# graphdeco-inria/hierarchical-3d-gaussians

Hardware: AMD Instinct MI355X
Metric: fwd+bwd frames/s @1080p, 1M Gaussians (higher is better)
Workload: dtype f32

## Files before the change

hierarchical-3d-gaussians_amd/csrc/preprocess.hip:

```cpp
#include "gaussian_math.h"
#include "half_widen.h"

#include <stdlib.h>

#include <mutex>

namespace hgs {

namespace {

struct CamLds {
  float vm[16];
  float pm[16];
  float cam[3];
};

__device__ __forceinline__ void load_camera(const hgs_raster_args& a, CamLds& c) {
#pragma unroll
  for (int i = 0; i < 16; ++i) {
    c.vm[i] = a.viewmatrix[i];
    c.pm[i] = a.projmatrix[i];
  }
  c.cam[0] = a.campos[0];
  c.cam[1] = a.campos[1];
// ... 826 lines not shown
    for (int i = 0; i < 10; ++i) t[i] = 0.0;
#pragma unroll 4
    for (uint32_t k = (uint32_t)lane; k < r1 - r0; k += 64u) {
      const float2 v0 = ip[k * 5 + 0], v1 = ip[k * 5 + 1], v2 = ip[k * 5 + 2], v3 = ip[k * 5 + 3], v4 = ip[k * 5 + 4];
      t[0] += v0.x; t[1] += v0.y; t[2] += v1.x; t[3] += v1.y;
      t[4] += v2.x; t[5] += v2.y; t[6] += v3.x; t[7] += v3.y;
      t[8] += v4.x; t[9] += v4.y;
    }
#pragma unroll
    for (int i = 0; i < 10; ++i) red[i * 64 + lane] = t[i];
    __builtin_amdgcn_fence(__ATOMIC_RELEASE, "wavefront");
    __builtin_amdgcn_wave_barrier();
    __builtin_amdgcn_fence(__ATOMIC_ACQUIRE, "wavefront");
    if (lane < 40) {
      double acc = 0.0;
      const double* src = red + (lane >> 2) * 64 + (lane & 3) * 16;
#pragma unroll
      for (int j = 0; j < 16; ++j) acc += src[j];
      red[640 + lane] = acc;
    }
    __builtin_amdgcn_fence(__ATOMIC_RELEASE, "wavefront");
    __builtin_amdgcn_wave_barrier();
    __builtin_amdgcn_fence(__ATOMIC_ACQUIRE, "wavefront");
    if (lane < 10) {
      const double* q = red + 640 + lane * 4;
      reinterpret_cast<double*>(inst + rbase * kInstStride)[lane] = ((q[0] + q[1]) + q[2]) + q[3];
    }
    __builtin_amdgcn_fence(__ATOMIC_RELEASE, "wavefront");
    __builtin_amdgcn_wave_barrier();
  }
}

constexpr uint32_t kK8StageRec = 256;
__device__ __forceinline__ void k8_sum_runs(const GeomWs& g, const float* __restrict__ inst, int idx, uint32_t n,
                                            int presummed, float2* st, double (&s)[10]) {
  const int lane = threadIdx.x & 63;
  const unsigned long long long_mask = presummed ? __ballot(n > kK8LongRun) : 0ull;
  if (long_mask == 0ull) {
    uint32_t incl = n;
#pragma unroll
    for (int off = 1; off < 64; off <<= 1) {
      const uint32_t t = __shfl_up(incl, off, 64);
      if (lane >= off) incl += t;
    }
    const uint32_t my0 = incl - n, my1 = incl;
    const uint32_t total = __shfl(incl, 63, 64);
    if (total) {
      const unsigned long long nz = __ballot(n != 0u);
      const int first = __ffsll((long long)nz) - 1;
      const uint32_t off_mine = n ? g.offsets[idx] : 0u;
      const size_t base = (size_t)__shfl(off_mine, first, 64);
      for (uint32_t c0 = 0; c0 < total; c0 += kK8StageRec) {
        const uint32_t cn = min(kK8StageRec, total - c0) * 5u;
        const float2* src = reinterpret_cast<const float2*>(inst) + (base + c0) * 5;
        for (uint32_t t0 = 0; t0 < cn; t0 += 64u * 4u) {
          float2 v[4];
#pragma unroll
          for (int j = 0; j < 4; ++j) {
            const uint32_t t = t0 + (uint32_t)j * 64u + (uint32_t)lane;
            v[j] = src[min(t, cn - 1u)];
          }
#pragma unroll
          for (int j = 0; j < 4; ++j) {
            const uint32_t t = t0 + (uint32_t)j * 64u + (uint32_t)lane;
            if (t < cn) st[t] = v[j];
          }
        }
        __builtin_amdgcn_fence(__ATOMIC_RELEASE, "wavefront");
        __builtin_amdgcn_wave_barrier();
        __builtin_amdgcn_fence(__ATOMIC_ACQUIRE, "wavefront");
        const uint32_t k0 = max(my0, c0), k1 = min(my1, c0 + kK8StageRec);
        for (uint32_t k = k0; k < k1; ++k) {
          const float2* r = st + (k - c0) * 5u;
          const float2 v0 = r[0], v1 = r[1], v2 = r[2], v3 = r[3], v4 = r[4];
          s[0] += v0.x; s[1] += v0.y; s[2] += v1.x; s[3] += v1.y;
          s[4] += v2.x; s[5] += v2.y; s[6] += v3.x; s[7] += v3.y;
          s[8] += v4.x; s[9] += v4.y;
        }
        __builtin_amdgcn_fence(__ATOMIC_RELEASE, "wavefront");
        __builtin_amdgcn_wave_barrier();
      }
    }
  } else if (n != 0u) {
    const size_t off = (size_t)g.offsets[idx];
    if (n > kK8LongRun) {
      const uint32_t nseg = k8_nseg(n);
      for (uint32_t j = 0; j < nseg; ++j) {
        const double* ps = reinterpret_cast<const double*>(inst + (off + (size_t)j * kK8Seg) * kInstStride);
#pragma unroll
        for (int i = 0; i < 10; ++i) s[i] += ps[i];
      }
    } else {
      const float2* ip = reinterpret_cast<const float2*>(inst) + off * 5;
#pragma unroll 2
      for (uint32_t k = 0; k < n; ++k) {
        const float2 v0 = ip[k * 5 + 0], v1 = ip[k * 5 + 1], v2 = ip[k * 5 + 2], v3 = ip[k * 5 + 3], v4 = ip[k * 5 + 4];
        s[0] += v0.x; s[1] += v0.y; s[2] += v1.x; s[3] += v1.y;
        s[4] += v2.x; s[5] += v2.y; s[6] += v3.x; s[7] += v3.y;
        s[8] += v4.x; s[9] += v4.y;
      }
    }
  }
}

template <bool LOD>
__device__ __forceinline__ void k8_chain(const hgs_raster_args& a, const GeomWs& g, int idx, const double (&s)[10],
                                         float (&p)[3], float (&d_mean)[3], float (&d_m2)[3], float& d_op,
                                         float (&d_scale)[3], float (&d_rot)[4], float (&d_c3)[6], float (&gr)[3]) {
  CamLds cam;
  load_camera(a, cam);
  gr[0] = (float)s[6]; gr[1] = (float)s[7]; gr[2] = (float)s[8];
  const uint32_t flags = g.flags[idx];
  load_mean<LOD>(a, lod_row_gather<LOD>(a, idx), p);
  float q[4] = {1.f, 0.f, 0.f, 0.f};
  float sc[3] = {1.f, 1.f, 1.f};
  double qnorm = 1.0;
  ProjD pd;
  if (a.cov3D_precomp) {
#pragma unroll
    for (int i = 0; i < 6; ++i) pd.c3[i] = (double)a.cov3D_precomp[(size_t)idx * 6 + i];
  } else {
    load_scale_rot<LOD>(a, idx, sc, q, &qnorm);
    cov3d_from_scale_rot_d(sc, a.scale_modifier, q, pd);
  }
  project_gaussian_d(p, cam.vm, cam.pm, a.width, a.height, a.tanfovx, a.tanfovy, (flags & 8u) != 0,
                     (flags & 16u) != 0, pd);

  const double A = pd.conA, B = pd.conB, C = pd.conC;
  const double gA = -0.5 * s[2], gB = -s[3], gC = -0.5 * s[4];
  const double ggx = -(A * s[0] + B * s[1]);
  const double ggy = -(C * s[1] + B * s[0]);
  const double dm2x = ggx * 0.5 * (double)a.width, dm2y = ggy * 0.5 * (double)a.height;
  d_m2[0] = (float)dm2x;
  d_m2[1] = (float)dm2y;
  double dmean[3] = {0.0, 0.0, 0.0};

  const double dhx = dm2x * pd.pw, dhy = dm2y * pd.pw;
  const double dhw = -(dm2x * pd.hx + dm2y * pd.hy) * pd.pw * pd.pw;
#pragma unroll
  for (int j = 0; j < 3; ++j)
    dmean[j] += (double)cam.pm[j * 4 + 0] * dhx + (double)cam.pm[j * 4 + 1] * dhy + (double)cam.pm[j * 4 + 3] * dhw;

  const double a2 = pd.a, b2 = pd.b, c2 = pd.c;
  const double di2 = pd.di * pd.di;
  const double ga = (-c2 * c2 * gA + b2 * c2 * gB - b2 * b2 * gC) * di2;
  const double gb = (2.0 * b2 * c2 * gA - (a2 * c2 + b2 * b2) * gB + 2.0 * a2 * b2 * gC) * di2;
  const double gc = (-b2 * b2 * gA + a2 * b2 * gB - a2 * a2 * gC) * di2;
  const double hb = 0.5 * gb;
  double Gs[3][3];
#pragma unroll
  for (int i = 0; i < 3; ++i)
#pragma unroll
    for (int j = i; j < 3; ++j)
      Gs[i][j] = Gs[j][i] = pd.T0[i] * (ga * pd.T0[j] + hb * pd.T1[j]) + pd.T1[i] * (hb * pd.T0[j] + gc * pd.T1[j]);
  d_c3[0] = (float)Gs[0][0];
// ... 47 lines not shown
#pragma unroll
    for (int k = 0; k < 3; ++k) {
      double acc = 0.0;
#pragma unroll
      for (int i = 0; i < 3; ++i) {
        acc += R[i * 3 + k] * dM[i][k];
        gR[i][k] = dM[i][k] * sv[k];
      }
      double dsk = (double)a.scale_modifier * acc;
      if (a.activations & HGS_ACT_SCALE_EXP) dsk *= (double)sc[k];
      d_scale[k] = (float)dsk;
    }
    const double r = q[0], x = q[1], y = q[2], z = q[3];
    double dq[4];
    dq[0] = 2.0 * (-z * gR[0][1] + y * gR[0][2] + z * gR[1][0] - x * gR[1][2] - y * gR[2][0] + x * gR[2][1]);
    dq[1] = 2.0 * (y * gR[0][1] + z * gR[0][2] + y * gR[1][0] - 2.0 * x * gR[1][1] - r * gR[1][2] +
                   z * gR[2][0] + r * gR[2][1] - 2.0 * x * gR[2][2]);
    dq[2] = 2.0 * (-2.0 * y * gR[0][0] + x * gR[0][1] + r * gR[0][2] + x * gR[1][0] + z * gR[1][2] -
                   r * gR[2][0] + z * gR[2][1] - 2.0 * y * gR[2][2]);
    dq[3] = 2.0 * (-2.0 * z * gR[0][0] - r * gR[0][1] + x * gR[0][2] + r * gR[1][0] - 2.0 * z * gR[1][1] +
                   y * gR[1][2] + x * gR[2][0] + y * gR[2][1]);
    if (a.activations & HGS_ACT_ROT_NORMALIZE) {
      const double dot = r * dq[0] + x * dq[1] + y * dq[2] + z * dq[3];
      const double inv = 1.0 / qnorm;
      dq[0] = (dq[0] - r * dot) * inv; dq[1] = (dq[1] - x * dot) * inv;
      dq[2] = (dq[2] - y * dot) * inv; dq[3] = (dq[3] - z * dot) * inv;
    }
    d_rot[0] = (float)dq[0]; d_rot[1] = (float)dq[1]; d_rot[2] = (float)dq[2]; d_rot[3] = (float)dq[3];
  }

  {
    float dod = 1.0f;
    double dact = 1.0;
    const float o_act = load_opacity<LOD>(a, idx, &dact);
    float o_rec = o_act;
    if (a.interpolation_weights && a.num_node_kids && !a.lod_per_pixel)
      o_rec = lod_opacity(o_act, a.interpolation_weights[idx], a.num_node_kids[idx], &dod);
    const float sums5 = o_rec > 0.0f ? (float)(s[5] / (double)o_rec) : 0.0f;
    d_op = a.activations ? (float)((double)sums5 * (double)dod * dact) : sums5 * dod;
  }

  if (!a.colors_precomp) {
    if (flags & 1u) gr[0] = 0.f;
    if (flags & 2u) gr[1] = 0.f;
    if (flags & 4u) gr[2] = 0.f;
  }
}

template <bool ACC>
__device__ __forceinline__ void k8_store_row(const hgs_raster_grads& out, int idx, const float (&d_m2)[3], float d_op,
                                             const float (&d_scale)[3], const float (&d_rot)[4], const float (&d_c3)[6],
                                             const float (&d_col)[3]) {
  constexpr bool acc = ACC;
#pragma unroll
  for (int j = 0; j < 3; ++j) out.dL_dmeans2D[idx * 3 + j] = d_m2[j];
  out.dL_dopacity[idx] = d_op + (acc ? out.dL_dopacity[idx] : 0.f);
  if (out.dL_dcolors) {
#pragma unroll
    for (int j = 0; j < 3; ++j) out.dL_dcolors[idx * 3 + j] = d_col[j];
  }
  if (out.dL_dscales) {
#pragma unroll
    for (int j = 0; j < 3; ++j) out.dL_dscales[idx * 3 + j] = d_scale[j] + (acc ? out.dL_dscales[idx * 3 + j] : 0.f);
  }
  if (out.dL_drotations) {
    float4* dst = reinterpret_cast<float4*>(out.dL_drotations) + idx;
    float4 v = make_float4(d_rot[0], d_rot[1], d_rot[2], d_rot[3]);
    if (acc) { const float4 o = *dst; v.x += o.x; v.y += o.y; v.z += o.z; v.w += o.w; }
    *dst = v;
  }
  if (out.dL_dcov3D) {
#pragma unroll
    for (int j = 0; j < 6; ++j) out.dL_dcov3D[(size_t)idx * 6 + j] = d_c3[j] + (acc ? out.dL_dcov3D[(size_t)idx * 6 + j] : 0.f);
  }
}

template <bool ACC, bool LOD>
__global__ __launch_bounds__(kPreBlock) void preprocess_bwd_kernel(hgs_raster_args a, GeomWs g,
                                                                   const float* __restrict__ inst,
                                                                   float* __restrict__ drgb,
                                                                   float* __restrict__ dmean_rows,
                                                                   const uint32_t* __restrict__ lod_flag,
                                                                   hgs_raster_grads out, int presummed) {
  const int idx = blockIdx.x * kPreBlock + threadIdx.x;
  const bool in_range = idx < a.P;
  const uint32_t n = in_range ? g.tiles_touched[idx] : 0u;

  double s[10];
#pragma unroll
  for (int i = 0; i < 10; ++i) s[i] = 0.0;
  static_assert(kInstStride == 10, "instance record = the ten sums, 40 bytes");
  __shared__ float2 stage[kPreBlock / 64][kK8StageRec * 5];
  k8_sum_runs(g, inst, idx, n, presummed, stage[threadIdx.x >> 6], s);
  if constexpr (!LOD) {
    if (!in_range) return;
  }

  float d_mean[3] = {0.f, 0.f, 0.f};
  float d_m2[3] = {0.f, 0.f, 0.f};
  float d_op = 0.f;
  float d_scale[3] = {0.f, 0.f, 0.f};
  float d_rot[4] = {0.f, 0.f, 0.f, 0.f};
  float d_c3[6] = {0.f, 0.f, 0.f, 0.f, 0.f, 0.f};
  float gr[3] = {0.f, 0.f, 0.f};
  float d_col[3] = {0.f, 0.f, 0.f};
  if (n != 0) {
    float p[3];
    k8_chain<LOD>(a, g, idx, s, p, d_mean, d_m2, d_op, d_scale, d_rot, d_c3, gr);
    if (a.colors_precomp) {
      d_col[0] = gr[0]; d_col[1] = gr[1]; d_col[2] = gr[2];
    } else {
      drgb[idx * 3 + 0] = gr[0];
      drgb[idx * 3 + 1] = gr[1];
      drgb[idx * 3 + 2] = gr[2];
    }
  }

  if constexpr (LOD) {
    if (a.lod_scatter) {
      __shared__ float lds_v[8 * kPreBlock];
      __shared__ int lds_par[kPreBlock];
      __shared__ unsigned char lds_vis[kPreBlock];
      const int t = threadIdx.x;
      const int block_first = blockIdx.x * kPreBlock;
      const int count = min(kPreBlock, a.P - block_first);
      LodRow l;
      l.r = l.p = 0; l.w = 1.0f; l.u = 0.0f;
      if (in_range) l = lod_row<true>(a, idx);
      const bool self = l.p == l.r;
      const bool vis = in_range && n != 0;
      const float wn = self ? 1.0f : l.w, u = (self || !vis) ? 0.0f : l.u;
      float sgn = 1.0f;
      if (vis && !self && u != 0.0f) {
        const float4 qa = reinterpret_cast<const float4*>(a.rotations)[l.r];
        const float4 qb = reinterpret_cast<const float4*>(a.rotations)[l.p];
        sgn = (qa.x * qb.x + qa.y * qb.y + qa.z * qb.z + qa.w * qb.w) < 0.0f ? -1.0f : 1.0f;
      }
      if (in_range) {
#pragma unroll
        for (int j = 0; j < 3; ++j) {
          dmean_rows[idx * 3 + j] = d_mean[j];
          out.dL_dmeans2D[idx * 3 + j] = d_m2[j];
        }
      }
      if (vis) {
        out.dL_dopacity[l.r] = wn * d_op;
#pragma unroll
        for (int j = 0; j < 3; ++j) out.dL_dscales[l.r * 3 + j] = wn * d_scale[j];
        reinterpret_cast<float4*>(out.dL_drotations)[l.r] = make_float4(wn * d_rot[0], wn * d_rot[1], wn * d_rot[2], wn * d_rot[3]);
      }
      lds_par[t] = in_range ? (int)l.p : -1;
      lds_vis[t] = (vis && !self) ? 1 : 0;
#pragma unroll
      for (int j = 0; j < 3; ++j) lds_v[j * kPreBlock + t] = u * d_scale[j];
#pragma unroll
      for (int j = 0; j < 4; ++j) lds_v[(3 + j) * kPreBlock + t] = (u * sgn) * d_rot[j];
      lds_v[7 * kPreBlock + t] = u * d_op;
      __syncthreads();
      if (t < count) {
        const LodRun run = lod_run(a, lds_par, t, count, block_first, *lod_flag != 0u);
        if (run.leader) {
          float acc8[8] = {0.f, 0.f, 0.f, 0.f, 0.f, 0.f, 0.f, 0.f};
          bool any = false;
          for (int j = t; j < run.end; ++j) {
            if (!lds_vis[j]) continue;
            any = true;
#pragma unroll
            for (int k = 0; k < 8; ++k) acc8[k] += lds_v[k * kPreBlock + j];
          }
          if (any) {
            const size_t pp = (size_t)lds_par[t];
#pragma unroll
            for (int k = 0; k < 3; ++k) lod_add(out.dL_dscales + pp * 3 + k, acc8[k], run.atomic);
#pragma unroll
            for (int k = 0; k < 4; ++k) lod_add(out.dL_drotations + pp * 4 + k, acc8[3 + k], run.atomic);
            lod_add(out.dL_dopacity + pp, acc8[7], run.atomic);
          }
        }
      }
      return;
    }
    if (!in_range) return;
  }
#pragma unroll
  for (int j = 0; j < 3; ++j) out.dL_dmeans3D[idx * 3 + j] = d_mean[j] + (ACC ? out.dL_dmeans3D[idx * 3 + j] : 0.f);
  k8_store_row<ACC>(out, idx, d_m2, d_op, d_scale, d_rot, d_c3, d_col);
}


template <bool ACC, bool JAC, bool LOD>
__global__ __launch_bounds__(kPreBlock) void sh_bwd_kernel(hgs_raster_args a, GeomWs g,
                                                           const float* __restrict__ drgb,
                                                           const float* __restrict__ dmean_rows,
                                                           const uint32_t* __restrict__ lod_flag, hgs_raster_grads out) {
  extern __shared__ __attribute__((aligned(16))) unsigned char smem_raw[];
  float* lds = reinterpret_cast<float*>(smem_raw);
  const int n = a.M * 3;
  const bool split = a.shs_rest != nullptr;
  const bool coop = (n & 3) == 0;
  const int block_first = blockIdx.x * kPreBlock;
  const int idx = block_first + threadIdx.x;
  const bool valid = idx < a.P;
  const bool active = valid && g.tiles_touched[idx] != 0;
  if (!JAC && coop) {
    if (split) {
      coop_load_seg(a.shs, block_first, a.P, 3, 0, sh_row_stride(n), lds);
      coop_load_seg(a.shs_rest, block_first, a.P, n - 3, 3, sh_row_stride(n), lds);
    } else {
      coop_load_sh(a.shs, block_first, a.P, n, lds);
    }
    __syncthreads();
  }
  float dsh[48];
#pragma unroll
  for (int i = 0; i < 48; ++i) dsh[i] = 0.f;
  float sh[JAC ? 1 : 48];
  if constexpr (!JAC) {
    if (active) {
      if (coop) lds_row_read(lds, n, sh);
// ... 143 lines not shown
    float* d1 = out.dL_dshs_rest + (size_t)idx * (n - 3);
#pragma unroll
    for (int i = 0; i < 48; ++i) {
      if (i < 3) d0[i] = dsh[i] + (ACC ? d0[i] : 0.f);
      else if (i < n) d1[i - 3] = dsh[i] + (ACC ? d1[i - 3] : 0.f);
    }
  } else if (valid) {
    if (ACC) {
      const float* old = out.dL_dshs + (size_t)idx * n;
#pragma unroll
      for (int i = 0; i < 48; ++i)
        if (i < n) dsh[i] += old[i];
    }
    store_sh(out.dL_dshs, idx, a.M, dsh);
  }
}

__device__ __forceinline__ float k8_dot3(float x0, float y0, float x1, float y1, float x2, float y2) {
#pragma clang fp contract(off)
  return __fmaf_rn(x2, y2, __fmaf_rn(x0, y0, x1 * y1));
}
__device__ __forceinline__ void k8_add_view_term(const float (&gr)[3], const float (&J)[9], float ux, float uy, float uz,
                                                 float inv, float (&d_mean)[3]) {
#pragma clang fp contract(off)
  const float gdx = k8_dot3(gr[0], J[0], gr[1], J[1], gr[2], J[2]);
  const float gdy = k8_dot3(gr[0], J[3], gr[1], J[4], gr[2], J[5]);
  const float gdz = k8_dot3(gr[0], J[6], gr[1], J[7], gr[2], J[8]);
  const float dot = k8_dot3(ux, gdx, uy, gdy, uz, gdz);
  d_mean[0] = __fmaf_rn(__fmaf_rn(-ux, dot, gdx), inv, d_mean[0] + 0.f);
  d_mean[1] = __fmaf_rn(__fmaf_rn(-uy, dot, gdy), inv, d_mean[1] + 0.f);
  d_mean[2] = __fmaf_rn(__fmaf_rn(-uz, dot, gdz), inv, d_mean[2] + 0.f);
}

__global__ __launch_bounds__(kPreBlock) void preprocess_bwd_sh_kernel(hgs_raster_args a, GeomWs g,
                                                                         const float* __restrict__ inst,
                                                                         hgs_raster_grads out, int presummed) {
  extern __shared__ __attribute__((aligned(16))) unsigned char smem_raw[];
  const int block_first = blockIdx.x * kPreBlock;
  const int idx = block_first + threadIdx.x;
  const bool in_range = idx < a.P;
  const uint32_t n = in_range ? g.tiles_touched[idx] : 0u;

  double s[10];
#pragma unroll
  for (int i = 0; i < 10; ++i) s[i] = 0.0;
  k8_sum_runs(g, inst, idx, n, presummed, reinterpret_cast<float2*>(smem_raw) + (threadIdx.x >> 6) * (kK8StageRec * 5), s);

  float d_mean[3] = {0.f, 0.f, 0.f};
  float d_m2[3] = {0.f, 0.f, 0.f};
  float d_op = 0.f;
  float d_scale[3] = {0.f, 0.f, 0.f};
  float d_rot[4] = {0.f, 0.f, 0.f, 0.f};
  float d_c3[6] = {0.f, 0.f, 0.f, 0.f, 0.f, 0.f};
  float gr[3] = {0.f, 0.f, 0.f};
  float b[16];
  const int nb = (a.sh_degree + 1) * (a.sh_degree + 1);
  float p[3];
  if (n != 0) k8_chain<false>(a, g, idx, s, p, d_mean, d_m2, d_op, d_scale, d_rot, d_c3, gr);
  if (in_range) {
    const float d_col[3] = {0.f, 0.f, 0.f};
    k8_store_row<false>(out, idx, d_m2, d_op, d_scale, d_rot, d_c3, d_col);
  }
  __builtin_amdgcn_sched_barrier(0);
  if (n != 0) {
    float ux, uy, uz;
    const float inv = unit_dir(p, a.campos, ux, uy, uz);
    sh_basis(a.sh_degree, ux, uy, uz, b);
    const float* jp = g.shjac + (size_t)idx * kJacStride;
    float J[9];
#pragma unroll
    for (int k = 0; k < 9; ++k) J[k] = jp[k];
    k8_add_view_term(gr, J, ux, uy, uz, inv, d_mean);
  } else {
#pragma unroll
    for (int j = 0; j < 3; ++j) d_mean[j] = 0.f;
  }
  if (in_range) {
#pragma unroll
    for (int j = 0; j < 3; ++j) out.dL_dmeans3D[idx * 3 + j] = d_mean[j];
  }

  float* lds = reinterpret_cast<float*>(smem_raw);
  const int nc = a.M * 3, stride = sh_row_stride(nc);
  __syncthreads();
  if (in_range) {
    float* row = lds + threadIdx.x * stride;
#pragma unroll
    for (int i = 0; i < 12; ++i) {
      if (i * 4 < nc) {
        float v[4];
#pragma unroll
        for (int c = 0; c < 4; ++c) {
          const int k = (i * 4 + c) / 3, ch = (i * 4 + c) % 3;
          v[c] = (n != 0 && k < nb) ? b[k] * gr[ch] : 0.f;
        }
        *reinterpret_cast<float4*>(row + i * 4) = make_float4(v[0], v[1], v[2], v[3]);
      }
    }
  }
  __syncthreads();
  coop_store_sh<false>(out.dL_dshs, block_first, a.P, nc, lds);
}

template <bool ACC, bool COOP, bool COLOR>
__device__ __forceinline__ void sh_bwd_batched_body(const ShBwdViews& v, int P, int M, int sh_degree,
                                                    const float* __restrict__ means3D, const float* __restrict__ shs,
                                                    float* __restrict__ dL_dshs, float* __restrict__ dL_dmeans3D) {
  extern __shared__ __attribute__((aligned(16))) unsigned char smem_raw[];
  float* lds = reinterpret_cast<float*>(smem_raw);
  const int n = M * 3;
  constexpr bool coop = COOP;
  const int block_first = blockIdx.x * kPreBlock;
// ... 250 lines not shown
              : h48   ? (jac ? preprocess_fwd_h48_kernel<true> : preprocess_fwd_h48_kernel<false>)
              : defer ? (jac ? preprocess_fwd_kernel<true, false, true> : preprocess_fwd_kernel<false, false, true>)
                      : (jac ? preprocess_fwd_kernel<true, false, false> : preprocess_fwd_kernel<false, false, false>);
    hipLaunchKernelGGL(k1, dim3(nblk), dim3(kPreBlock), lds_bytes, s, a, g, radii, super, heavy_thr);
    HGS_LAUNCH_CHECK("preprocess_fwd", s, a.debug);
  }
  return HGS_OK;
}

int launch_scan_block_sums(const GeomWs& g, int32_t P, hipStream_t s, bool debug, uint32_t* total_mirror) {
  const int nblk = (P + kPreBlock - 1) / kPreBlock;
  const int chunks = scan_chunks(nblk), resident = scan_resident_workgroups();
  if (chunks * (1 + kBands) <= resident && !scan_split_forced()) {
    hipLaunchKernelGGL(scan_block_sums_kernel, dim3(chunks, 1 + kBands), dim3(1024), 0, s, g.block_sums, g.block_band,
                       nblk, g.scan_chain, total_mirror, 0, chunks);
    HGS_LAUNCH_CHECK("scan_block_sums", s, debug);
    return HGS_OK;
  }
  for (int y = 0; y < 1 + kBands; ++y) {
    uint32_t* sums = y == 0 ? g.block_sums : g.block_band + (size_t)(y - 1) * (nblk + 1);
    for (int c0 = 0; c0 < chunks; c0 += resident) {
      hipLaunchKernelGGL(scan_block_sums_kernel, dim3(min(resident, chunks - c0), 1), dim3(1024), 0, s, sums, g.block_band,
                         nblk, g.scan_chain + (size_t)y * chunks, y == 0 ? total_mirror : nullptr, c0, chunks);
      HGS_LAUNCH_CHECK("scan_block_sums", s, debug);
    }
  }
  return HGS_OK;
}

int launch_preprocess_bwd(const hgs_raster_args& a, const GeomWs& g, const BwdWs& w, const hgs_raster_grads& out, uint32_t L,
                          hipStream_t s) {
  const int nblk = (a.P + kPreBlock - 1) / kPreBlock;
  if (nblk > 0) {
    static const char* force = getenv("HGS_K8_PRESUM");
    const bool presum = force ? force[0] == '1' : (uint64_t)L > 6ull * (uint64_t)a.P;
    if (presum) {
      HGS_HIP(hipMemsetAsync(w.work_counter, 0, sizeof(uint32_t), s));
      hipLaunchKernelGGL(k8_worklist_kernel, dim3(nblk < kWorklistGrid ? nblk : kWorklistGrid), dim3(kPreBlock), 0, s, a.P,
                         g.tiles_touched, w.work, w.work_counter);
      HGS_LAUNCH_CHECK("preprocess_bwd_worklist", s, a.debug);
      const int want = (int)(((size_t)L / 64 + 3) / 4);
      hipLaunchKernelGGL(k8_presum_work_kernel, dim3(want < 1 ? 1 : (want < kPresumGrid ? want : kPresumGrid)), dim3(kPreBlock), 0,
                         s, w.work, w.work_counter, g.tiles_touched, g.offsets, w.inst_grads);
      HGS_LAUNCH_CHECK("preprocess_bwd_long_runs", s, a.debug);
    }
    const char* fuse_env = getenv("HGS_K8_FUSE");
    const bool fused = !(fuse_env && fuse_env[0] == '0') && !a.lod_render_indices && !a.accumulate_grads &&
                       !a.defer_sh_bwd && a.shs && !a.shs_rest && out.dL_dshs && a.prepare_backward && !a.colors_precomp &&
                       ((a.M * 3) & 3) == 0;
    if (fused) {
      const size_t stage_bytes = (size_t)(kPreBlock / 64) * kK8StageRec * 5 * sizeof(float2);
      const size_t rows_bytes = (size_t)kPreBlock * (a.M * 3 + 4) * sizeof(float);
      hipLaunchKernelGGL(preprocess_bwd_sh_kernel, dim3(nblk), dim3(kPreBlock),
                         stage_bytes > rows_bytes ? stage_bytes : rows_bytes, s, a, g, w.inst_grads, out, presum ? 1 : 0);
      HGS_LAUNCH_CHECK("preprocess_bwd_sh", s, a.debug);
      return HGS_OK;
    }
    auto k8a = a.lod_render_indices ? preprocess_bwd_kernel<false, true>
                                    : (a.accumulate_grads ? preprocess_bwd_kernel<true, false> : preprocess_bwd_kernel<false, false>);
    hipLaunchKernelGGL(k8a, dim3(nblk), dim3(kPreBlock), 0, s, a, g, w.inst_grads, w.drgb, w.dmean_rows, w.lod_flag, out,
                       presum ? 1 : 0);
    HGS_LAUNCH_CHECK("preprocess_bwd", s, a.debug);
    if (a.shs && out.dL_dshs && !a.defer_sh_bwd) {
      const size_t lds_bytes = (size_t)kPreBlock * (a.M * 3 + 4) * sizeof(float);
      auto k8b = a.lod_render_indices ? sh_bwd_kernel<false, true, true>
                 : (a.prepare_backward && a.shs) ? (a.accumulate_grads ? sh_bwd_kernel<true, true, false> : sh_bwd_kernel<false, true, false>)
                                                 : (a.accumulate_grads ? sh_bwd_kernel<true, false, false> : sh_bwd_kernel<false, false, false>);
      hipLaunchKernelGGL(k8b, dim3(nblk), dim3(kPreBlock), lds_bytes, s, a, g, w.drgb, w.dmean_rows, w.lod_flag, out);
      HGS_LAUNCH_CHECK("sh_bwd", s, a.debug);
    }
  }
  return HGS_OK;
}

}
```

Measured before the change: 1529.

## Stage backward preprocess inputs and instance grads into LDS via direct global-to-LDS loads

Adds a staged variant of the per-Gaussian backward preprocess kernels. Per-instance gradient records, per-Gaussian means, scales, rotations, opacity, flags and the SH Jacobian rows are loaded into LDS with global_load_lds (buffer-to-LDS DMA) instead of going through VGPRs. The camera load is hoisted to kernel entry and the row store in the fused kernel is moved to the end, so the loads can overlap the summation. The new path raises LDS use per block, which may reduce occupancy. It also depends on 16-byte alignment checks, shifted-offset arithmetic and explicit vmcnt waits.

```diff
diff --git a/hierarchical-3d-gaussians_amd/csrc/k8a_body.h b/hierarchical-3d-gaussians_amd/csrc/k8a_body.h
--- /dev/null
+++ b/hierarchical-3d-gaussians_amd/csrc/k8a_body.h
@@ -0,0 +1,115 @@
+  const int idx = blockIdx.x * kPreBlock + threadIdx.x;
+  const bool in_range = idx < a.P;
+  static_assert(kInstStride == 10, "instance record = the ten sums, 40 bytes");
+  __shared__ __attribute__((aligned(16))) float2 stage[kPreBlock / 64][kK8StageRec * 5];
+  __shared__ __attribute__((aligned(16))) unsigned char staged_in[STG ? (kPreBlock / 64) * kK8InWave : 16];
+  const int wave = threadIdx.x >> 6;
+  const unsigned char* in = staged_in + (STG ? wave * kK8InWave : 0);
+  CamLds cam;
+  if constexpr (STG) {
+    load_camera(a, cam);
+    k8_stage_inputs(a, g, idx, mode, staged_in + wave * kK8InWave);
+  }
+  const uint32_t n = in_range ? g.tiles_touched[idx] : 0u;
+  uint32_t off = 0u;
+  if constexpr (STG) { if (in_range) off = g.offsets[idx]; }
+  else { if (n) off = g.offsets[idx]; }
+
+  double s[10];
+#pragma unroll
+  for (int i = 0; i < 10; ++i) s[i] = 0.0;
+  k8_sum_runs<STG>(inst, off, n, mode, stage[wave], s);
+  if constexpr (STG) asm volatile("s_waitcnt vmcnt(0)" ::: "memory");
+  if constexpr (!LOD) {
+    if (!in_range) return;
+  }
+
+  float d_mean[3] = {0.f, 0.f, 0.f};
+  float d_m2[3] = {0.f, 0.f, 0.f};
+  float d_op = 0.f;
+  float d_scale[3] = {0.f, 0.f, 0.f};
+  float d_rot[4] = {0.f, 0.f, 0.f, 0.f};
+  float d_c3[6] = {0.f, 0.f, 0.f, 0.f, 0.f, 0.f};
+  float gr[3] = {0.f, 0.f, 0.f};
+  float d_col[3] = {0.f, 0.f, 0.f};
+  if (n != 0) {
+    float p[3];
+    k8_chain<LOD, STG>(a, g, idx, s, p, d_mean, d_m2, d_op, d_scale, d_rot, d_c3, gr, in, &cam);
+    if (a.colors_precomp) {
+      d_col[0] = gr[0]; d_col[1] = gr[1]; d_col[2] = gr[2];
+    } else {
+      drgb[idx * 3 + 0] = gr[0];
+      drgb[idx * 3 + 1] = gr[1];
+      drgb[idx * 3 + 2] = gr[2];
+    }
+  }
+
+  if constexpr (LOD) {
+    if (a.lod_scatter) {
+      __shared__ float lds_v[8 * kPreBlock];
+      __shared__ int lds_par[kPreBlock];
+      __shared__ unsigned char lds_vis[kPreBlock];
+      const int t = threadIdx.x;
+      const int block_first = blockIdx.x * kPreBlock;
+      const int count = min(kPreBlock, a.P - block_first);
+      LodRow l;
+      l.r = l.p = 0; l.w = 1.0f; l.u = 0.0f;
+      if (in_range) l = lod_row<true>(a, idx);
+      const bool self = l.p == l.r;
+      const bool vis = in_range && n != 0;
+      const float wn = self ? 1.0f : l.w, u = (self || !vis) ? 0.0f : l.u;
+      float sgn = 1.0f;
+      if (vis && !self && u != 0.0f) {
+        const float4 qa = reinterpret_cast<const float4*>(a.rotations)[l.r];
+        const float4 qb = reinterpret_cast<const float4*>(a.rotations)[l.p];
+        sgn = (qa.x * qb.x + qa.y * qb.y + qa.z * qb.z + qa.w * qb.w) < 0.0f ? -1.0f : 1.0f;
+      }
+      if (in_range) {
+#pragma unroll
+        for (int j = 0; j < 3; ++j) {
+          dmean_rows[idx * 3 + j] = d_mean[j];
+          out.dL_dmeans2D[idx * 3 + j] = d_m2[j];
+        }
+      }
+      if (vis) {
+        out.dL_dopacity[l.r] = wn * d_op;
+#pragma unroll
+        for (int j = 0; j < 3; ++j) out.dL_dscales[l.r * 3 + j] = wn * d_scale[j];
+        reinterpret_cast<float4*>(out.dL_drotations)[l.r] = make_float4(wn * d_rot[0], wn * d_rot[1], wn * d_rot[2], wn * d_rot[3]);
+      }
+      lds_par[t] = in_range ? (int)l.p : -1;
+      lds_vis[t] = (vis && !self) ? 1 : 0;
+#pragma unroll
+      for (int j = 0; j < 3; ++j) lds_v[j * kPreBlock + t] = u * d_scale[j];
+#pragma unroll
+      for (int j = 0; j < 4; ++j) lds_v[(3 + j) * kPreBlock + t] = (u * sgn) * d_rot[j];
+      lds_v[7 * kPreBlock + t] = u * d_op;
+      __syncthreads();
+      if (t < count) {
+        const LodRun run = lod_run(a, lds_par, t, count, block_first, *lod_flag != 0u);
+        if (run.leader) {
+          float acc8[8] = {0.f, 0.f, 0.f, 0.f, 0.f, 0.f, 0.f, 0.f};
+          bool any = false;
+          for (int j = t; j < run.end; ++j) {
+            if (!lds_vis[j]) continue;
+            any = true;
+#pragma unroll
+            for (int k = 0; k < 8; ++k) acc8[k] += lds_v[k * kPreBlock + j];
+          }
+          if (any) {
+            const size_t pp = (size_t)lds_par[t];
+#pragma unroll
+            for (int k = 0; k < 3; ++k) lod_add(out.dL_dscales + pp * 3 + k, acc8[k], run.atomic);
+#pragma unroll
+            for (int k = 0; k < 4; ++k) lod_add(out.dL_drotations + pp * 4 + k, acc8[3 + k], run.atomic);
+            lod_add(out.dL_dopacity + pp, acc8[7], run.atomic);
+          }
+        }
+      }
+      return;
+    }
+    if (!in_range) return;
+  }
+#pragma unroll
+  for (int j = 0; j < 3; ++j) out.dL_dmeans3D[idx * 3 + j] = d_mean[j] + (ACC ? out.dL_dmeans3D[idx * 3 + j] : 0.f);
+  k8_store_row<ACC>(out, idx, d_m2, d_op, d_scale, d_rot, d_c3, d_col);
diff --git a/hierarchical-3d-gaussians_amd/csrc/preprocess.hip b/hierarchical-3d-gaussians_amd/csrc/preprocess.hip
--- a/hierarchical-3d-gaussians_amd/csrc/preprocess.hip
+++ b/hierarchical-3d-gaussians_amd/csrc/preprocess.hip
@@ -882,9 +882,57 @@
 }
 
 constexpr uint32_t kK8StageRec = 256;
-__device__ __forceinline__ void k8_sum_runs(const GeomWs& g, const float* __restrict__ inst, int idx, uint32_t n,
-                                            int presummed, float2* st, double (&s)[10]) {
+constexpr uint32_t kK8StageBytes = kK8StageRec * kInstStride * 4;
+constexpr uint32_t kK8DmaRec = 254;
+static_assert((8 + kK8DmaRec * kInstStride * 4 + 15) / 16 <= kK8StageBytes / 16,
+              "a DMA pass, shifted, fits the stage in whole 16-byte pieces");
+constexpr int kK8ModePresum = 1, kK8ModeStage = 2, kK8ModeStageIn = 4;
+constexpr uint32_t kK8InWave = 64 * (12 + 12 + 16 + 4 + 4);
+constexpr uint32_t kK8InMean = 0, kK8InScale = 768, kK8InRot = 1536, kK8InOp = 2560, kK8InFlags = 2816;
+constexpr uint32_t kK8LdsBytes = (kPreBlock / 64) * (kK8StageBytes + kK8InWave);
+
+__host__ __device__ __forceinline__ uint32_t k8_pass_shift(size_t first) { return (uint32_t)((first * (kInstStride * 4)) & 15u); }
+__host__ __device__ __forceinline__ uint32_t k8_pass_pieces(size_t first, uint32_t cnt) {
+  return (k8_pass_shift(first) + cnt * (kInstStride * 4) + 15u) >> 4;
+}
+
+__device__ __forceinline__ void k8_stage_inputs(const hgs_raster_args& a, const GeomWs& g, int idx, int mode, unsigned char* in) {
+  const int lane = threadIdx.x & 63, wave_first = idx & ~63;
+  const bool sr = !a.cov3D_precomp;
+  if ((mode & kK8ModeStageIn) && wave_first + 64 <= a.P) {
+    const char* m = reinterpret_cast<const char*>(a.means3D + (size_t)wave_first * 3);
+    const char* o = reinterpret_cast<const char*>(a.opacities + wave_first);
+    const char* f = reinterpret_cast<const char*>(g.flags + wave_first);
+    if (lane < 48) __builtin_amdgcn_global_load_lds((gptr_t)(m + lane * 16), (lptr_t)(in + kK8InMean), 16, 0, 0);
+    if (sr) {
+      const char* sc = reinterpret_cast<const char*>(a.scales + (size_t)wave_first * 3);
+      const char* r = reinterpret_cast<const char*>(a.rotations + (size_t)wave_first * 4);
+      if (lane < 48) __builtin_amdgcn_global_load_lds((gptr_t)(sc + lane * 16), (lptr_t)(in + kK8InScale), 16, 0, 0);
+      __builtin_amdgcn_global_load_lds((gptr_t)(r + lane * 16), (lptr_t)(in + kK8InRot), 16, 0, 0);
+    }
+    if (lane < 16) {
+      __builtin_amdgcn_global_load_lds((gptr_t)(o + lane * 16), (lptr_t)(in + kK8InOp), 16, 0, 0);
+      __builtin_amdgcn_global_load_lds((gptr_t)(f + lane * 16), (lptr_t)(in + kK8InFlags), 16, 0, 0);
+    }
+  } else if (idx < a.P) {
+    float* m = reinterpret_cast<float*>(in + kK8InMean) + lane * 3;
+    m[0] = a.means3D[idx * 3 + 0]; m[1] = a.means3D[idx * 3 + 1]; m[2] = a.means3D[idx * 3 + 2];
+    if (sr) {
+      float* sc = reinterpret_cast<float*>(in + kK8InScale) + lane * 3;
+      sc[0] = a.scales[idx * 3 + 0]; sc[1] = a.scales[idx * 3 + 1]; sc[2] = a.scales[idx * 3 + 2];
+      reinterpret_cast<float4*>(in + kK8InRot)[lane] = reinterpret_cast<const float4*>(a.rotations)[idx];
+    }
+    reinterpret_cast<float*>(in + kK8InOp)[lane] = a.opacities[idx];
+    reinterpret_cast<uint32_t*>(in + kK8InFlags)[lane] = g.flags[idx];
+  }
+}
+
+template <bool STG>
+__device__ __forceinline__ void k8_sum_runs(const float* __restrict__ inst, uint32_t off, uint32_t n,
+                                            int mode, float2* st, double (&s)[10]) {
   const int lane = threadIdx.x & 63;
+  const int presummed = mode & kK8ModePresum;
+  constexpr bool dma = STG;
   const unsigned long long long_mask = presummed ? __ballot(n > kK8LongRun) : 0ull;
   if (long_mask == 0ull) {
     uint32_t incl = n;
@@ -898,30 +946,45 @@
     if (total) {
       const unsigned long long nz = __ballot(n != 0u);
       const int first = __ffsll((long long)nz) - 1;
-      const uint32_t off_mine = n ? g.offsets[idx] : 0u;
-      const size_t base = (size_t)__shfl(off_mine, first, 64);
-      for (uint32_t c0 = 0; c0 < total; c0 += kK8StageRec) {
-        const uint32_t cn = min(kK8StageRec, total - c0) * 5u;
-        const float2* src = reinterpret_cast<const float2*>(inst) + (base + c0) * 5;
-        for (uint32_t t0 = 0; t0 < cn; t0 += 64u * 4u) {
-          float2 v[4];
-#pragma unroll
-          for (int j = 0; j < 4; ++j) {
-            const uint32_t t = t0 + (uint32_t)j * 64u + (uint32_t)lane;
-            v[j] = src[min(t, cn - 1u)];
+      const size_t base = (size_t)__shfl(n ? off : 0u, first, 64);
+      const uint32_t pass = dma ? kK8DmaRec : kK8StageRec;
+      for (uint32_t c0 = 0; c0 < total; c0 += pass) {
+        const uint32_t cnt = min(pass, total - c0);
+        uint32_t shift2 = 0;
+        if (dma) {
+          const uint32_t shift = k8_pass_shift(base + c0), pieces = k8_pass_pieces(base + c0, cnt);
+          const char* src = reinterpret_cast<const char*>(inst) + ((base + c0) * (kInstStride * 4) - shift);
+#pragma unroll
+          for (uint32_t j = 0; j < kK8StageBytes / 1024; ++j) {
+            const uint32_t piece = j * 64u + (uint32_t)lane;
+            if (piece < pieces)
+              __builtin_amdgcn_global_load_lds((gptr_t)(src + (size_t)piece * 16), (lptr_t)(reinterpret_cast<char*>(st) + j * 1024), 16, 0, 0);
           }
-#pragma unroll
-          for (int j = 0; j < 4; ++j) {
-            const uint32_t t = t0 + (uint32_t)j * 64u + (uint32_t)lane;
-            if (t < cn) st[t] = v[j];
+          asm volatile("s_waitcnt vmcnt(0)" ::: "memory");
+          shift2 = shift >> 3;
+        } else {
+          const uint32_t cn = cnt * 5u;
+          const float2* src = reinterpret_cast<const float2*>(inst) + (base + c0) * 5;
+          for (uint32_t t0 = 0; t0 < cn; t0 += 64u * 4u) {
+            float2 v[4];
+#pragma unroll
+            for (int j = 0; j < 4; ++j) {
+              const uint32_t t = t0 + (uint32_t)j * 64u + (uint32_t)lane;
+              v[j] = src[min(t, cn - 1u)];
+            }
+#pragma unroll
+            for (int j = 0; j < 4; ++j) {
+              const uint32_t t = t0 + (uint32_t)j * 64u + (uint32_t)lane;
+              if (t < cn) st[t] = v[j];
+            }
           }
         }
         __builtin_amdgcn_fence(__ATOMIC_RELEASE, "wavefront");
         __builtin_amdgcn_wave_barrier();
         __builtin_amdgcn_fence(__ATOMIC_ACQUIRE, "wavefront");
-        const uint32_t k0 = max(my0, c0), k1 = min(my1, c0 + kK8StageRec);
+        const uint32_t k0 = max(my0, c0), k1 = min(my1, c0 + pass);
         for (uint32_t k = k0; k < k1; ++k) {
-          const float2* r = st + (k - c0) * 5u;
+          const float2* r = st + shift2 + (k - c0) * 5u;
           const float2 v0 = r[0], v1 = r[1], v2 = r[2], v3 = r[3], v4 = r[4];
           s[0] += v0.x; s[1] += v0.y; s[2] += v1.x; s[3] += v1.y;
           s[4] += v2.x; s[5] += v2.y; s[6] += v3.x; s[7] += v3.y;
@@ -932,16 +995,15 @@
       }
     }
   } else if (n != 0u) {
-    const size_t off = (size_t)g.offsets[idx];
     if (n > kK8LongRun) {
       const uint32_t nseg = k8_nseg(n);
       for (uint32_t j = 0; j < nseg; ++j) {
-        const double* ps = reinterpret_cast<const double*>(inst + (off + (size_t)j * kK8Seg) * kInstStride);
+        const double* ps = reinterpret_cast<const double*>(inst + ((size_t)off + (size_t)j * kK8Seg) * kInstStride);
 #pragma unroll
         for (int i = 0; i < 10; ++i) s[i] += ps[i];
       }
     } else {
-      const float2* ip = reinterpret_cast<const float2*>(inst) + off * 5;
+      const float2* ip = reinterpret_cast<const float2*>(inst) + (size_t)off * 5;
 #pragma unroll 2
       for (uint32_t k = 0; k < n; ++k) {
         const float2 v0 = ip[k * 5 + 0], v1 = ip[k * 5 + 1], v2 = ip[k * 5 + 2], v3 = ip[k * 5 + 3], v4 = ip[k * 5 + 4];
@@ -953,15 +1015,27 @@
   }
 }
 
-template <bool LOD>
+template <bool LOD, bool STG>
 __device__ __forceinline__ void k8_chain(const hgs_raster_args& a, const GeomWs& g, int idx, const double (&s)[10],
                                          float (&p)[3], float (&d_mean)[3], float (&d_m2)[3], float& d_op,
-                                         float (&d_scale)[3], float (&d_rot)[4], float (&d_c3)[6], float (&gr)[3]) {
-  CamLds cam;
-  load_camera(a, cam);
+                                         float (&d_scale)[3], float (&d_rot)[4], float (&d_c3)[6], float (&gr)[3],
+                                         const unsigned char* in, const CamLds* cam_entry) {
+  CamLds cam_here;
+  if constexpr (!STG) load_camera(a, cam_here);
+  const CamLds& cam = STG ? *cam_entry : cam_here;
   gr[0] = (float)s[6]; gr[1] = (float)s[7]; gr[2] = (float)s[8];
-  const uint32_t flags = g.flags[idx];
-  load_mean<LOD>(a, lod_row_gather<LOD>(a, idx), p);
+  const int lane = threadIdx.x & 63;
+  static_assert(!(LOD && STG), "the LOD route gathers rows by index");
+  constexpr bool staged = STG;
+  uint32_t flags;
+  if (staged) {
+    flags = reinterpret_cast<const uint32_t*>(in + kK8InFlags)[lane];
+    const float* m = reinterpret_cast<const float*>(in + kK8InMean) + lane * 3;
+    p[0] = m[0]; p[1] = m[1]; p[2] = m[2];
+  } else {
+    flags = g.flags[idx];
+    load_mean<LOD>(a, lod_row_gather<LOD>(a, idx), p);
+  }
   float q[4] = {1.f, 0.f, 0.f, 0.f};
   float sc[3] = {1.f, 1.f, 1.f};
   double qnorm = 1.0;
@@ -970,7 +1044,23 @@
 #pragma unroll
     for (int i = 0; i < 6; ++i) pd.c3[i] = (double)a.cov3D_precomp[(size_t)idx * 6 + i];
   } else {
-    load_scale_rot<LOD>(a, idx, sc, q, &qnorm);
+    if (staged) {
+      const float* sr = reinterpret_cast<const float*>(in + kK8InScale) + lane * 3;
+      sc[0] = sr[0]; sc[1] = sr[1]; sc[2] = sr[2];
+      if (a.activations & HGS_ACT_SCALE_EXP) {
+#pragma unroll
+        for (int i = 0; i < 3; ++i) sc[i] = (float)exp((double)sc[i]);
+      }
+      const float4 qv = reinterpret_cast<const float4*>(in + kK8InRot)[lane];
+      q[0] = qv.x; q[1] = qv.y; q[2] = qv.z; q[3] = qv.w;
+      if (a.activations & HGS_ACT_ROT_NORMALIZE) {
+        const double w = q[0], x = q[1], y = q[2], z = q[3];
+        qnorm = fmax(sqrt(((w * w + x * x) + y * y) + z * z), 1e-12);
+        q[0] = (float)(w / qnorm); q[1] = (float)(x / qnorm); q[2] = (float)(y / qnorm); q[3] = (float)(z / qnorm);
+      }
+    } else {
+      load_scale_rot<LOD>(a, idx, sc, q, &qnorm);
+    }
     cov3d_from_scale_rot_d(sc, a.scale_modifier, q, pd);
   }
   project_gaussian_d(p, cam.vm, cam.pm, a.width, a.height, a.tanfovx, a.tanfovy, (flags & 8u) != 0,
@@ -1084,7 +1174,21 @@
   {
     float dod = 1.0f;
     double dact = 1.0;
-    const float o_act = load_opacity<LOD>(a, idx, &dact);
+    float o_act;
+    if (staged) {
+      const float raw = reinterpret_cast<const float*>(in + kK8InOp)[lane];
+      o_act = raw;
+      if (a.activations & HGS_ACT_OPACITY_SIGMOID) {
+        const double o = 1.0 / (1.0 + exp(-(double)raw));
+        dact = o * (1.0 - o);
+        o_act = (float)o;
+      } else if (a.activations & HGS_ACT_OPACITY_ABS) {
+        dact = raw > 0.f ? 1.0 : (raw < 0.f ? -1.0 : 0.0);
+        o_act = fabsf(raw);
+      }
+    } else {
+      o_act = load_opacity<LOD>(a, idx, &dact);
+    }
     float o_rec = o_act;
     if (a.interpolation_weights && a.num_node_kids && !a.lod_per_pixel)
       o_rec = lod_opacity(o_act, a.interpolation_weights[idx], a.num_node_kids[idx], &dod);
@@ -1133,110 +1237,19 @@
                                                                    float* __restrict__ drgb,
                                                                    float* __restrict__ dmean_rows,
                                                                    const uint32_t* __restrict__ lod_flag,
-                                                                   hgs_raster_grads out, int presummed) {
-  const int idx = blockIdx.x * kPreBlock + threadIdx.x;
-  const bool in_range = idx < a.P;
-  const uint32_t n = in_range ? g.tiles_touched[idx] : 0u;
-
-  double s[10];
-#pragma unroll
-  for (int i = 0; i < 10; ++i) s[i] = 0.0;
-  static_assert(kInstStride == 10, "instance record = the ten sums, 40 bytes");
-  __shared__ float2 stage[kPreBlock / 64][kK8StageRec * 5];
-  k8_sum_runs(g, inst, idx, n, presummed, stage[threadIdx.x >> 6], s);
-  if constexpr (!LOD) {
-    if (!in_range) return;
-  }
-
-  float d_mean[3] = {0.f, 0.f, 0.f};
-  float d_m2[3] = {0.f, 0.f, 0.f};
-  float d_op = 0.f;
-  float d_scale[3] = {0.f, 0.f, 0.f};
-  float d_rot[4] = {0.f, 0.f, 0.f, 0.f};
-  float d_c3[6] = {0.f, 0.f, 0.f, 0.f, 0.f, 0.f};
-  float gr[3] = {0.f, 0.f, 0.f};
-  float d_col[3] = {0.f, 0.f, 0.f};
-  if (n != 0) {
-    float p[3];
-    k8_chain<LOD>(a, g, idx, s, p, d_mean, d_m2, d_op, d_scale, d_rot, d_c3, gr);
-    if (a.colors_precomp) {
-      d_col[0] = gr[0]; d_col[1] = gr[1]; d_col[2] = gr[2];
-    } else {
-      drgb[idx * 3 + 0] = gr[0];
-      drgb[idx * 3 + 1] = gr[1];
-      drgb[idx * 3 + 2] = gr[2];
-    }
-  }
-
-  if constexpr (LOD) {
-    if (a.lod_scatter) {
-      __shared__ float lds_v[8 * kPreBlock];
-      __shared__ int lds_par[kPreBlock];
-      __shared__ unsigned char lds_vis[kPreBlock];
-      const int t = threadIdx.x;
-      const int block_first = blockIdx.x * kPreBlock;
-      const int count = min(kPreBlock, a.P - block_first);
-      LodRow l;
-      l.r = l.p = 0; l.w = 1.0f; l.u = 0.0f;
-      if (in_range) l = lod_row<true>(a, idx);
-      const bool self = l.p == l.r;
-      const bool vis = in_range && n != 0;
-      const float wn = self ? 1.0f : l.w, u = (self || !vis) ? 0.0f : l.u;
-      float sgn = 1.0f;
-      if (vis && !self && u != 0.0f) {
-        const float4 qa = reinterpret_cast<const float4*>(a.rotations)[l.r];
-        const float4 qb = reinterpret_cast<const float4*>(a.rotations)[l.p];
-        sgn = (qa.x * qb.x + qa.y * qb.y + qa.z * qb.z + qa.w * qb.w) < 0.0f ? -1.0f : 1.0f;
-      }
-      if (in_range) {
-#pragma unroll
-        for (int j = 0; j < 3; ++j) {
-          dmean_rows[idx * 3 + j] = d_mean[j];
-          out.dL_dmeans2D[idx * 3 + j] = d_m2[j];
-        }
-      }
-      if (vis) {
-        out.dL_dopacity[l.r] = wn * d_op;
-#pragma unroll
-        for (int j = 0; j < 3; ++j) out.dL_dscales[l.r * 3 + j] = wn * d_scale[j];
-        reinterpret_cast<float4*>(out.dL_drotations)[l.r] = make_float4(wn * d_rot[0], wn * d_rot[1], wn * d_rot[2], wn * d_rot[3]);
-      }
-      lds_par[t] = in_range ? (int)l.p : -1;
-      lds_vis[t] = (vis && !self) ? 1 : 0;
-#pragma unroll
-      for (int j = 0; j < 3; ++j) lds_v[j * kPreBlock + t] = u * d_scale[j];
-#pragma unroll
-      for (int j = 0; j < 4; ++j) lds_v[(3 + j) * kPreBlock + t] = (u * sgn) * d_rot[j];
-      lds_v[7 * kPreBlock + t] = u * d_op;
-      __syncthreads();
-      if (t < count) {
-        const LodRun run = lod_run(a, lds_par, t, count, block_first, *lod_flag != 0u);
-        if (run.leader) {
-          float acc8[8] = {0.f, 0.f, 0.f, 0.f, 0.f, 0.f, 0.f, 0.f};
-          bool any = false;
-          for (int j = t; j < run.end; ++j) {
-            if (!lds_vis[j]) continue;
-            any = true;
-#pragma unroll
-            for (int k = 0; k < 8; ++k) acc8[k] += lds_v[k * kPreBlock + j];
-          }
-          if (any) {
-            const size_t pp = (size_t)lds_par[t];
-#pragma unroll
-            for (int k = 0; k < 3; ++k) lod_add(out.dL_dscales + pp * 3 + k, acc8[k], run.atomic);
-#pragma unroll
-            for (int k = 0; k < 4; ++k) lod_add(out.dL_drotations + pp * 4 + k, acc8[3 + k], run.atomic);
-            lod_add(out.dL_dopacity + pp, acc8[7], run.atomic);
-          }
-        }
-      }
-      return;
-    }
-    if (!in_range) return;
-  }
-#pragma unroll
-  for (int j = 0; j < 3; ++j) out.dL_dmeans3D[idx * 3 + j] = d_mean[j] + (ACC ? out.dL_dmeans3D[idx * 3 + j] : 0.f);
-  k8_store_row<ACC>(out, idx, d_m2, d_op, d_scale, d_rot, d_c3, d_col);
+                                                                   hgs_raster_grads out, int mode) {
+  constexpr bool STG = false;
+#include "k8a_body.h"
+}
+template <bool ACC>
+__global__ __launch_bounds__(kPreBlock) void preprocess_bwd_staged_kernel(hgs_raster_args a, GeomWs g,
+                                                                          const float* __restrict__ inst,
+                                                                          float* __restrict__ drgb,
+                                                                          float* __restrict__ dmean_rows,
+                                                                          const uint32_t* __restrict__ lod_flag,
+                                                                          hgs_raster_grads out, int mode) {
+  constexpr bool LOD = false, STG = true;
+#include "k8a_body.h"
 }
 
 
@@ -1446,19 +1459,43 @@
   d_mean[2] = __fmaf_rn(__fmaf_rn(-uz, dot, gdz), inv, d_mean[2] + 0.f);
 }
 
+template <bool STG>
 __global__ __launch_bounds__(kPreBlock) void preprocess_bwd_sh_kernel(hgs_raster_args a, GeomWs g,
                                                                          const float* __restrict__ inst,
-                                                                         hgs_raster_grads out, int presummed) {
+                                                                         hgs_raster_grads out, int mode) {
   extern __shared__ __attribute__((aligned(16))) unsigned char smem_raw[];
   const int block_first = blockIdx.x * kPreBlock;
   const int idx = block_first + threadIdx.x;
   const bool in_range = idx < a.P;
+  const int wave = threadIdx.x >> 6, wave_first = idx & ~63;
+  unsigned char* st = smem_raw + wave * kK8StageBytes;
+  unsigned char* in = smem_raw + (kPreBlock / 64) * kK8StageBytes + wave * kK8InWave;
+  CamLds cam;
+  if constexpr (STG) {
+    load_camera(a, cam);
+    k8_stage_inputs(a, g, idx, mode, in);
+  }
   const uint32_t n = in_range ? g.tiles_touched[idx] : 0u;
+  uint32_t off = 0u;
+  if constexpr (STG) { if (in_range) off = g.offsets[idx]; }
+  else { if (n) off = g.offsets[idx]; }
 
   double s[10];
 #pragma unroll
   for (int i = 0; i < 10; ++i) s[i] = 0.0;
-  k8_sum_runs(g, inst, idx, n, presummed, reinterpret_cast<float2*>(smem_raw) + (threadIdx.x >> 6) * (kK8StageRec * 5), s);
+  k8_sum_runs<STG>(inst, off, n, mode, reinterpret_cast<float2*>(st), s);
+  const bool jac_staged = STG && wave_first < a.P;
+  if constexpr (STG) {
+    asm volatile("s_waitcnt vmcnt(0)" ::: "memory");
+    if (jac_staged) {
+      const int lane = threadIdx.x & 63;
+      const char* src = reinterpret_cast<const char*>(g.shjac + (size_t)wave_first * kJacStride);
+      static_assert(64 * kJacStride * 4 == 2304, "64 Jacobian rows = 144 pieces of 16 bytes");
+      __builtin_amdgcn_global_load_lds((gptr_t)(src + lane * 16), (lptr_t)st, 16, 0, 0);
+      __builtin_amdgcn_global_load_lds((gptr_t)(src + 1024 + lane * 16), (lptr_t)(st + 1024), 16, 0, 0);
+      if (lane < 16) __builtin_amdgcn_global_load_lds((gptr_t)(src + 2048 + lane * 16), (lptr_t)(st + 2048), 16, 0, 0);
+    }
+  }
 
   float d_mean[3] = {0.f, 0.f, 0.f};
   float d_m2[3] = {0.f, 0.f, 0.f};
@@ -1470,20 +1507,28 @@
   float b[16];
   const int nb = (a.sh_degree + 1) * (a.sh_degree + 1);
   float p[3];
-  if (n != 0) k8_chain<false>(a, g, idx, s, p, d_mean, d_m2, d_op, d_scale, d_rot, d_c3, gr);
-  if (in_range) {
+  if (n != 0) k8_chain<false, STG>(a, g, idx, s, p, d_mean, d_m2, d_op, d_scale, d_rot, d_c3, gr, in, &cam);
+  constexpr bool stores_last = STG;
+  if (in_range && !stores_last) {
     const float d_col[3] = {0.f, 0.f, 0.f};
     k8_store_row<false>(out, idx, d_m2, d_op, d_scale, d_rot, d_c3, d_col);
   }
   __builtin_amdgcn_sched_barrier(0);
+  if constexpr (STG) asm volatile("s_waitcnt vmcnt(0)" ::: "memory");
   if (n != 0) {
     float ux, uy, uz;
-    const float inv = unit_dir(p, a.campos, ux, uy, uz);
+    const float inv = unit_dir(p, STG ? cam.cam : a.campos, ux, uy, uz);
     sh_basis(a.sh_degree, ux, uy, uz, b);
-    const float* jp = g.shjac + (size_t)idx * kJacStride;
     float J[9];
-#pragma unroll
-    for (int k = 0; k < 9; ++k) J[k] = jp[k];
+    if (jac_staged) {
+      const float* jl = reinterpret_cast<const float*>(st) + (threadIdx.x & 63) * kJacStride;
+#pragma unroll
+      for (int k = 0; k < 9; ++k) J[k] = jl[k];
+    } else {
+      const float* jp = g.shjac + (size_t)idx * kJacStride;
+#pragma unroll
+      for (int k = 0; k < 9; ++k) J[k] = jp[k];
+    }
     k8_add_view_term(gr, J, ux, uy, uz, inv, d_mean);
   } else {
 #pragma unroll
@@ -1492,6 +1537,10 @@
   if (in_range) {
 #pragma unroll
     for (int j = 0; j < 3; ++j) out.dL_dmeans3D[idx * 3 + j] = d_mean[j];
+    if (stores_last) {
+      const float d_col[3] = {0.f, 0.f, 0.f};
+      k8_store_row<false>(out, idx, d_m2, d_op, d_scale, d_rot, d_c3, d_col);
+    }
   }
 
   float* lds = reinterpret_cast<float*>(smem_raw);
@@ -1808,7 +1857,7 @@
                           hipStream_t s) {
   const int nblk = (a.P + kPreBlock - 1) / kPreBlock;
   if (nblk > 0) {
-    static const char* force = getenv("HGS_K8_PRESUM");
+    const char* force = getenv("HGS_K8_PRESUM");
     const bool presum = force ? force[0] == '1' : (uint64_t)L > 6ull * (uint64_t)a.P;
     if (presum) {
       HGS_HIP(hipMemsetAsync(w.work_counter, 0, sizeof(uint32_t), s));
@@ -1820,22 +1869,31 @@
                          s, w.work, w.work_counter, g.tiles_touched, g.offsets, w.inst_grads);
       HGS_LAUNCH_CHECK("preprocess_bwd_long_runs", s, a.debug);
     }
+    const char* stage_env = getenv("HGS_K8_STAGE");
+    const auto al16 = [](const void* p) { return (reinterpret_cast<uintptr_t>(p) & 15u) == 0; };
+    int mode = presum ? kK8ModePresum : 0;
+    if (!(stage_env && stage_env[0] == '0') && !a.lod_render_indices && al16(w.inst_grads) && al16(g.shjac)) {
+      mode |= kK8ModeStage;
+      if (al16(a.means3D) && al16(a.scales) && al16(a.rotations) && al16(a.opacities) && al16(g.flags)) mode |= kK8ModeStageIn;
+    }
+    const bool stg = (mode & kK8ModeStage) != 0;
     const char* fuse_env = getenv("HGS_K8_FUSE");
     const bool fused = !(fuse_env && fuse_env[0] == '0') && !a.lod_render_indices && !a.accumulate_grads &&
                        !a.defer_sh_bwd && a.shs && !a.shs_rest && out.dL_dshs && a.prepare_backward && !a.colors_precomp &&
                        ((a.M * 3) & 3) == 0;
     if (fused) {
-      const size_t stage_bytes = (size_t)(kPreBlock / 64) * kK8StageRec * 5 * sizeof(float2);
+      const size_t stage_bytes = kK8LdsBytes;
       const size_t rows_bytes = (size_t)kPreBlock * (a.M * 3 + 4) * sizeof(float);
-      hipLaunchKernelGGL(preprocess_bwd_sh_kernel, dim3(nblk), dim3(kPreBlock),
-                         stage_bytes > rows_bytes ? stage_bytes : rows_bytes, s, a, g, w.inst_grads, out, presum ? 1 : 0);
+      hipLaunchKernelGGL(stg ? preprocess_bwd_sh_kernel<true> : preprocess_bwd_sh_kernel<false>, dim3(nblk), dim3(kPreBlock),
+                         stage_bytes > rows_bytes ? stage_bytes : rows_bytes, s, a, g, w.inst_grads, out, mode);
       HGS_LAUNCH_CHECK("preprocess_bwd_sh", s, a.debug);
       return HGS_OK;
     }
     auto k8a = a.lod_render_indices ? preprocess_bwd_kernel<false, true>
-                                    : (a.accumulate_grads ? preprocess_bwd_kernel<true, false> : preprocess_bwd_kernel<false, false>);
+               : stg ? (a.accumulate_grads ? preprocess_bwd_staged_kernel<true> : preprocess_bwd_staged_kernel<false>)
+                     : (a.accumulate_grads ? preprocess_bwd_kernel<true, false> : preprocess_bwd_kernel<false, false>);
     hipLaunchKernelGGL(k8a, dim3(nblk), dim3(kPreBlock), 0, s, a, g, w.inst_grads, w.drgb, w.dmean_rows, w.lod_flag, out,
-                       presum ? 1 : 0);
+                       mode);
     HGS_LAUNCH_CHECK("preprocess_bwd", s, a.debug);
     if (a.shs && out.dL_dshs && !a.defer_sh_bwd) {
       const size_t lds_bytes = (size_t)kPreBlock * (a.M * 3 + 4) * sizeof(float);
```

New measurement: 1555 (median of 6 runs). +1.7%, better.
